# bensonlzl/spaced-kmer-sketching

Measured on AMD Instinct MI355X. Metric: k-mers hashed/s + genome-pairs ANI/s at 1/2/4/8 MI355X; % HBM roofline, higher is better.
Workload: dtype u64; 1 GPU; config3: 1x3 Gb multi-contig genome per GPU, spaced seed w=31/k=21 (mask seed 0), FracMinHash 1/1000; builds_in_flight=3, genome_bytes=3000000024, windows_per_genome=2999036400, sketch_size=2998764, parallelism=genome-sharded x1

## Files before the change

### include/sks.h

```cpp
#ifndef SKS_H
#define SKS_H

#include <stddef.h>
#include <stdint.h>

#ifdef __cplusplus
extern "C" {
#endif

#define SKS_ABI_VERSION 3

typedef enum sks_status {
  SKS_OK = 0,
  SKS_E_ARG = 1,
  SKS_E_HIP = 2,
  SKS_E_IO = 3,
  SKS_E_NOMEM = 4,
  SKS_E_UNSUPPORTED = 5,
  SKS_E_LENGTH = 6
} sks_status;

typedef enum sks_policy_kind {
  SKS_FRAC_MOD = 0,
  SKS_BOTTOM_S = 1
// ... 172 lines not shown
int sks_ani_matrix(sks_ctx* ctx, const int32_t* d_counts, uint32_t n, int kmer_num_ones, double* d_cont,
                   double* d_ani);
int sks_ani_rows(sks_ctx* ctx, const int32_t* d_counts, uint32_t n, uint32_t row_begin, uint32_t row_end,
                 int kmer_num_ones, double* d_cont, double* d_ani);
int sks_ani_tiles(sks_ctx* ctx, const int32_t* d_packed, const uint32_t* d_tiles, uint64_t n_tiles, uint32_t n,
                  const int32_t* d_sizes, int kmer_num_ones, double* d_ani);

int sks_fasta_parse_device(sks_ctx* ctx, const uint8_t* d_raw, uint64_t n_raw, uint8_t* d_stream,
                           uint64_t stream_cap, uint64_t* d_rec_end, uint64_t rec_cap,
                           uint64_t* stream_bytes, uint64_t* n_records);
int sks_ctx_last_ingress_ms(sks_ctx* ctx, float* ms);

int sks_ctx_last_intersect_ms(sks_ctx* ctx, float* ms);
int sks_ctx_set_scan_grid(sks_ctx* ctx, int grid);
enum {
  SKS_INTERSECT_AUTO = 0,
  SKS_INTERSECT_MERGE = 1,
  SKS_INTERSECT_JOIN = 2,
  SKS_INTERSECT_GLOBAL = 3
};
int sks_ctx_set_intersect_kernel(sks_ctx* ctx, int kind);
int sks_ctx_set_join_check(sks_ctx* ctx, int on);
int sks_ctx_join_check_violations(sks_ctx* ctx, uint64_t* violations);

int sks_synth_bases(sks_ctx* ctx, uint8_t* d_out, uint64_t n, uint64_t seed, uint64_t mut_seed,
                    double mut_rate, uint64_t pos_offset);

#ifdef __cplusplus
}
#endif
// ... 2 lines not shown
```

### spaced-kmer-sketching_amd/csrc/api.cpp

```cpp
#include <hip/hip_runtime.h>

#include <algorithm>
#include <cmath>
#include <cstdlib>
#include <cstring>
#include <mutex>
#include <numeric>
#include <random>
#include <string>
#include <thread>
#include <vector>

#include "sks.h"
#include "sks_api_internal.hpp"
#include "sks_hash.hpp"
#include "sks_ani.hpp"
#include "sks_internal.hpp"

namespace sks {

thread_local std::string g_last_error;

int fail(int code, const std::string& msg) {
  g_last_error = msg;
// ... 160 lines not shown
  sks::Scratch rec[3];
  sks::Scratch buf[10];
  sks::Scratch flag, pos;
  sks::Scratch meta;
  sks::Scratch iwork;
  sks::Scratch tdone;
  sks::Scratch lay;
  const uint32_t* layout_stat = nullptr;
  std::vector<uint64_t> meta_host;
  sks_timings last{};
  int grid_override = 0;
  int intersect_algo = 0;
  bool join_check = false;
  uint32_t layout_blocks_hint = 0;
  sks::Scratch root;
  uint32_t root_size = 0;
  int root_k = 0;
};

struct sks_kmer_list {
  int device = 0;
  uint32_t n = 0;
  uint64_t total = 0;
  uint64_t* d_pos = nullptr;
  uint64_t* d_bits = nullptr;
  std::vector<uint64_t> counts;
};


namespace {
// ... 151 lines not shown
      } else {
        ++i;
      }
    }
  }
  for (const CachedBlock& b : drop) {
    if (b.ready) (void)hipEventDestroy(b.ready);
    (void)hipFree(b.p);
  }
}

void release_set_arrays(sks_sketch_set* set, hipStream_t stream, bool ordered) {
  uint64_t total = 0;
  for (uint32_t v : set->sizes) total += v;
  void* arrays[3] = {set->d_data, set->d_starts, set->d_sizes};
  const size_t bytes[3] = {std::max<uint64_t>(total * set->elem_words, 1) * 8,
                           (size_t)std::max<uint32_t>(set->n, 1) * 8,
                           (size_t)std::max<uint32_t>(set->n, 1) * 4};
  for (int i = 0; i < 3; ++i) {
    if (!arrays[i]) continue;
    hipEvent_t ev = nullptr;
    if (ordered) {
      if (hipEventCreateWithFlags(&ev, hipEventDisableTiming) != hipSuccess ||
          hipEventRecord(ev, stream) != hipSuccess) {
        if (ev) (void)hipEventDestroy(ev);
        ev = nullptr;
        (void)hipGetLastError();
        (void)hipStreamSynchronize(stream);
      }
    }
    dev_release(arrays[i], bytes[i], ev);
// ... 140 lines not shown
  if (!out) return sks::fail(SKS_E_ARG, "sks_ctx_create: null out");
  *out = nullptr;
  int n = 0;
  hipError_t e = hipGetDeviceCount(&n);
  if (e != hipSuccess || n == 0)
    return sks::fail(SKS_E_HIP, std::string("sks_ctx_create: no HIP device available (the engine has "
                                            "no CPU path): hipGetDeviceCount -> ") +
                                    hipGetErrorString(e) + ", " + std::to_string(n) + " devices");
  if (device < 0 || device >= n) return sks::fail(SKS_E_ARG, "sks_ctx_create: bad device index");
  DeviceGuard g(device);
  sks_ctx* c = new (std::nothrow) sks_ctx();
  if (!c) return sks::fail(SKS_E_NOMEM, "sks_ctx_create: out of memory");
  c->device = device;
  c->stream = reinterpret_cast<hipStream_t>(stream);
  for (sks::Scratch* sc : {&c->ingress, &c->tmp, &c->rec[0], &c->rec[1], &c->rec[2], &c->flag,
                           &c->pos, &c->meta, &c->iwork, &c->tdone, &c->lay, &c->root})
    sc->owner = &c->stream;
  for (auto& b : c->buf) b.owner = &c->stream;
  if (hipEventCreate(&c->ev_begin) != hipSuccess || hipEventCreate(&c->ev_end) != hipSuccess ||
      hipEventCreate(&c->ev_s0) != hipSuccess || hipEventCreate(&c->ev_s1) != hipSuccess ||
      hipEventCreate(&c->ev_i0) != hipSuccess || hipEventCreate(&c->ev_i1) != hipSuccess) {
    delete c;
    return sks::fail(SKS_E_HIP, "sks_ctx_create: hipEventCreate failed");
  }
#define SKS_CALL_HOOK(tu) \
  if (e == hipSuccess) e = sks::code_object_hook_##tu(c->stream);
  e = hipSuccess;
  SKS_TU_LIST(SKS_CALL_HOOK)
#undef SKS_CALL_HOOK
  if (e != hipSuccess) {
    delete c;
// ... 5 lines not shown

int sks_ctx_destroy(sks_ctx* c) {
  if (!c) return SKS_OK;
  DeviceGuard g(c->device);
  (void)hipStreamSynchronize(c->stream);
  c->tmp.release();
  for (auto& r : c->rec) r.release();
  for (auto& b : c->buf) b.release();
  c->flag.release();
  c->pos.release();
  c->meta.release();
  c->iwork.release();
  c->tdone.release();
  c->lay.release();
  c->root.release();
  c->ingress.release();
  trim_device_cache(c->device);
  (void)hipEventDestroy(c->ev_begin);
  (void)hipEventDestroy(c->ev_end);
  (void)hipEventDestroy(c->ev_s0);
  (void)hipEventDestroy(c->ev_s1);
  if (c->ev_i0) (void)hipEventDestroy(c->ev_i0);
  if (c->ev_i1) (void)hipEventDestroy(c->ev_i1);
  delete c;
  return SKS_OK;
}

int sks_ctx_device(const sks_ctx* c) { return c ? c->device : -1; }

int sks_ctx_set_stream(sks_ctx* c, void* stream) {
// ... 12 lines not shown
  SKS_HIP(hipStreamSynchronize(c->stream));
  return SKS_OK;
}

int sks_ctx_last_timings(const sks_ctx* c, sks_timings* out) {
  if (!c || !out) return sks::fail(SKS_E_ARG, "sks_ctx_last_timings: null argument");
  *out = c->last;
  return SKS_OK;
}

int sks_ctx_set_scan_grid(sks_ctx* c, int grid) {
  if (!c) return sks::fail(SKS_E_ARG, "null ctx");
  c->grid_override = grid;
  return SKS_OK;
}

int sks_ctx_set_intersect_kernel(sks_ctx* c, int kind) {
  if (!c) return sks::fail(SKS_E_ARG, "null ctx");
  if (kind < SKS_INTERSECT_AUTO || kind > SKS_INTERSECT_GLOBAL)
    return sks::fail(SKS_E_ARG, "sks_ctx_set_intersect_kernel: unknown kernel");
  c->intersect_algo = kind;
  return SKS_OK;
}

int sks_ctx_set_layout_blocks_hint(sks_ctx* c, uint32_t blocks) {
  if (!c) return sks::fail(SKS_E_ARG, "sks_ctx_set_layout_blocks_hint: null ctx");
  c->layout_blocks_hint = blocks;
  return SKS_OK;
}

// ... 407 lines not shown
  tm.total_ms = tot;
  tm.post_ms = tot - ms;
  set->elem_words = 1;
  set->sizes = {(uint32_t)size};
  set->starts = {0};
  set->windows = {windows};
  set->window = S.w;
  set->mask[0] = S.mask_lo;
  set->mask[1] = S.mask_hi;
  set->policy = S.pol;
  c->last = tm;
  *out = set;
  return SKS_OK;
}

int validate_build(const char* fn, sks_ctx* c, const uint8_t* d_seq, uint64_t n_bytes,
                   const uint64_t* seg_off, uint32_t n_seg, int window, const uint64_t mask[2],
                   const sks_policy* policy) {
  const std::string f(fn);
  if (!c || !mask || !policy || (!seg_off && n_seg)) return sks::fail(SKS_E_ARG, f + ": null argument");
  if (window < 1 || window > 64)
    return sks::fail(SKS_E_ARG, f + ": window must be in [1, 64] (MAX_KMER_LENGTH)");
  if (policy->kind != SKS_FRAC_MOD && policy->kind != SKS_BOTTOM_S)
    return sks::fail(SKS_E_ARG, f + ": unknown policy kind");
  if (policy->flavour != 0 && policy->flavour != 1)
    return sks::fail(SKS_E_ARG, f + ": unknown hash flavour");
  if (policy->param == 0) return sks::fail(SKS_E_ARG, f + ": policy param must be > 0");
  {
    const int bits = 2 * window;
    uint64_t lo_allowed = bits >= 64 ? ~0ull : ((1ull << bits) - 1);
// ... 19 lines not shown
                     uint32_t n_seg, int window, const uint64_t mask[2], const sks_policy* policy,
                     sks_sketch_set** out) {
  if (!out) return sks::fail(SKS_E_ARG, "sks_sketch_build: null argument");
  *out = nullptr;
  SKS_TRY(validate_build("sks_sketch_build", c, d_seq, n_bytes, seg_off, n_seg, window, mask, policy));

  DeviceGuard guard(c->device);
  hipStream_t st = c->stream;
  BuildState S{c, window, window > 32, window > 32 ? 2 : 1, mask[0], mask[1], *policy,
               sks::fmh_const(mask[0], mask[1], window, policy->nonce, policy->flavour), {}};
  if (policy->kind == SKS_FRAC_MOD) S.dt = sks::make_div_test(policy->param);
  const bool bottom = policy->kind == SKS_BOTTOM_S;
  const double alpha = 1.0 + 10.0 / std::sqrt((double)policy->param) + 1.0 / (double)policy->param;

  sks_timings tm{};
  SKS_HIP(hipEventRecord(c->ev_begin, st));

  std::vector<uint64_t> thresh_g(n_seg, ~0ull), cap_g(n_seg), windows_g(n_seg, 0);
  std::vector<uint64_t> final_size(n_seg, ~0ull);
  for (uint32_t g = 0; g < n_seg; ++g) {
    const uint64_t L = seg_off[g + 1] - seg_off[g];
    double expect;
    if (!bottom) {
      expect = (double)L / (double)policy->param;
    } else {
      double want = alpha * (double)policy->param;
      if ((double)L <= want) {
        thresh_g[g] = ~0ull;
        expect = (double)L;
      } else {
// ... 5 lines not shown
    double cap = expect + 6.0 * std::sqrt(expect) + 4096.0;
    cap_g[g] = (uint64_t)std::min<double>(cap, (double)L + 1.0);
  }

  if (bottom && !S.wide && n_seg == 1 && getenv("SKS_NO_FAST_BOTTOM") == nullptr) {
    const uint64_t L = seg_off[1] - seg_off[0];
    const double expect = std::min<double>((double)L, alpha * (double)policy->param);
    const uint64_t cap = std::min<uint64_t>(cap_g[0], (uint64_t)(expect + 8.0 * std::sqrt(expect) + 256.0));
    if (L > 0 && cap <= sks::bottom_fused_capacity()) {
      const int rc = build_bottom_single(S, d_seq, seg_off, thresh_g[0], cap, tm, out);
      if (rc != kFastFallback) return rc;
      tm = sks_timings{};
    }
  }

  std::vector<PassOut> passes;
  std::vector<uint32_t> pending(n_seg);
  std::iota(pending.begin(), pending.end(), 0);
  int guard_passes = 0;
  while (!pending.empty()) {
    if (++guard_passes > 64) {
      free_passes(passes);
      return sks::fail(SKS_E_HIP, "sks_sketch_build: selection did not converge");
    }
    const uint32_t m = (uint32_t)pending.size();
    std::vector<uint64_t> beg(m), end(m), tp(m + 1, 0), thr(m), cap(m), ooff(m);
    uint64_t total_cap = 0;
    for (uint32_t i = 0; i < m; ++i) {
      uint32_t g = pending[i];
      beg[i] = seg_off[g];
      end[i] = seg_off[g + 1];
      tp[i + 1] = tp[i] + sks::scan_tiles_for(end[i] - beg[i]);
      thr[i] = thresh_g[g];
      cap[i] = cap_g[g];
      ooff[i] = total_cap;
      total_cap += cap[i];
    }
    const uint64_t n_tiles = tp[m];
    for (int r = 0; r < (bottom && S.wide ? 3 : (bottom || S.wide ? 2 : 1)); ++r)
      SKS_HIP(c->rec[r].reserve(std::max<uint64_t>(total_cap, 1) * sizeof(uint64_t)));
    MetaArena arena(c);
    size_t o_beg = arena.add(beg), o_end = arena.add(end), o_tp = arena.add(tp),
           o_thr = arena.add(thr), o_cap = arena.add(cap), o_off = arena.add(ooff),
           o_cnt = arena.add_zero(m), o_win = arena.add_zero(m), o_queue = arena.add_zero(1);
    SKS_TRY(arena.upload());

    const sks::ScanParams p = scan_params(S, d_seq, arena, o_beg, o_end, o_tp, o_thr, o_cap, o_off, o_cnt, o_win,
                                          m, n_tiles, o_queue);

    SKS_HIP(hipEventRecord(c->ev_s0, st));
    SKS_HIP(sks::launch_scan(p, bottom ? sks::kModeBottom : sks::kModeFrac, policy->flavour,
                             S.wide, c->device, st, c->grid_override));
    SKS_HIP(hipEventRecord(c->ev_s1, st));
    tm.scan_launches += n_tiles ? 1 : 0;
    if (o_win != o_cnt + m + 1) return sks::fail(SKS_E_HIP, "sks_sketch_build: arena layout");
    std::vector<uint64_t> cw(2 * (m + 1));
    SKS_HIP(sks::pinned_d2h(cw.data(), arena.ptr(o_cnt), cw.size() * sizeof(uint64_t), st));
    std::vector<uint64_t> counts(cw.begin(), cw.begin() + m), wins(cw.begin() + (m + 1), cw.begin() + (m + 1) + m);
    float ms = 0;
    SKS_HIP(hipEventElapsedTime(&ms, c->ev_s0, c->ev_s1));
    tm.scan_ms += ms;

    std::vector<uint32_t> ok, next;
    for (uint32_t i = 0; i < m; ++i) {
      tm.survivors += counts[i];
      if (counts[i] > cap[i]) {
        cap_g[pending[i]] = counts[i];
        next.push_back(pending[i]);
      } else {
        ok.push_back(i);
        windows_g[pending[i]] = wins[i];
      }
    }
    std::vector<uint32_t> retry_local;
    std::vector<uint64_t> fsz(m, ~0ull);
    int rc = post_process(S, pending, ooff, counts, thr, ok, passes, retry_local, fsz);
// ... 869 lines not shown
```

### spaced-kmer-sketching_amd/csrc/post.hip

```cpp
#include <hip/hip_runtime.h>

#include <algorithm>
#include <cstdio>
#include <cstring>
#include <rocprim/rocprim.hpp>
#include <rocprim/block/block_radix_sort.hpp>

#include "sks_hash.hpp"
#include "sks_internal.hpp"

namespace sks {

hipError_t Scratch::reserve(size_t n) {
  if (n <= bytes) return hipSuccess;
  const size_t grown = bytes + bytes / 2;
  if (ptr) {
    if (owner) {
      cache_release_after(ptr, bytes, *owner);
    } else {
      (void)hipDeviceSynchronize();
      (void)hipFree(ptr);
    }
  }
  ptr = nullptr;
// ... 674 lines not shown
  uint32_t eq_rank = block_excl_scan((uint32_t)__builtin_popcount(eq_m), wsum);
  uint32_t keep_m = lt_m;
#pragma unroll
  for (uint32_t j = 0; j < ITEMS; ++j)
    if ((eq_m >> j) & 1u) keep_m |= (eq_rank++ < sel.kk ? 1u : 0u) << j;
  uint32_t pos = block_excl_scan((uint32_t)__builtin_popcount(keep_m), wsum);
  uint64_t* skept = reinterpret_cast<uint64_t*>(smem);
#pragma unroll
  for (uint32_t j = 0; j < ITEMS; ++j)
    if ((keep_m >> j) & 1u) skept[pos++] = k[j];
  __syncthreads();
  for (uint32_t i = tid; i < (uint32_t)lim; i += kSelB) dst[i] = runs_expand(skept[i], runs);
  FSTAMP(7);
}

template <int FLAVOUR>
__global__ void k_fmh_narrow(uint64_t* __restrict__ keys, uint64_t n, uint64_t kconst) {
  const uint64_t i = (uint64_t)blockIdx.x * kB + threadIdx.x;
  if (i < n) keys[i] = hash_bitset128<FLAVOUR>(keys[i], 0) ^ kconst;
}

}

hipError_t seg_sort_keys(const uint64_t* keys_in, uint64_t* keys_out, uint64_t total,
                         const std::vector<uint64_t>& host_off, const uint64_t* d_off, int end_bit,
                         Scratch& tmp, hipStream_t s) {
  return sort_impl<false>(keys_in, keys_out, nullptr, nullptr, total, host_off, d_off, end_bit,
                          tmp, s);
}

// ... 237 lines not shown
      fprintf(stderr, "[k_bottom_fused stamps] n_seg %u max_cnt %llu: zero %llu count %llu scatter %llu isort %llu "
              "hash %llu distinct %llu select %llu write %llu\n", n_seg, (unsigned long long)max_cnt, h[0], h[1],
              h[2], h[3], h[4], h[5], h[6], h[7]);
    }
#endif
    return hipGetLastError();
  };
  if (max_cnt <= kSelB * 8)
    return flavour == 0 ? go(k_bottom_fused<0, 8>, fuse_lds<8>()) : go(k_bottom_fused<1, 8>, fuse_lds<8>());
  if (max_cnt <= kSelB * 12)
    return flavour == 0 ? go(k_bottom_fused<0, 12>, fuse_lds<12>())
                        : go(k_bottom_fused<1, 12>, fuse_lds<12>());
  return flavour == 0 ? go(k_bottom_fused<0, 16>, fuse_lds<16>()) : go(k_bottom_fused<1, 16>, fuse_lds<16>());
}

hipError_t launch_iota(uint64_t* out, uint64_t n, hipStream_t s) {
  if (n == 0) return hipSuccess;
  hipLaunchKernelGGL(k_iota, dim3(grid_for(n)), dim3(kB), 0, s, out, n);
  return hipGetLastError();
}

hipError_t launch_gather(const uint64_t* src, const uint64_t* idx, uint64_t n, uint64_t* out,
                         hipStream_t s) {
  if (n == 0) return hipSuccess;
  hipLaunchKernelGGL(k_gather, dim3(grid_for(n)), dim3(kB), 0, s, src, idx, n, out);
  return hipGetLastError();
}

hipError_t launch_interleave(const uint64_t* lo, const uint64_t* hi, uint64_t n, uint64_t* out,
                             hipStream_t s) {
// ... 9 lines not shown
```

### spaced-kmer-sketching_amd/csrc/sks_api_internal.hpp

```cpp
#pragma once
#include <cstdint>
#include <string>
#include <vector>

#include "sks.h"

struct sks_sketch_set {
  int device = 0;
  int elem_words = 1;
  uint32_t n = 0;
  uint64_t* d_data = nullptr;
  uint64_t* d_starts = nullptr;
  uint32_t* d_sizes = nullptr;
  std::vector<uint32_t> sizes;
  std::vector<uint64_t> starts;
  std::vector<uint64_t> windows;
  int window = 0;
  uint64_t mask[2] = {0, 0};
  sks_policy policy{};
  std::vector<std::string> names;
};

namespace sks {

int fail(int code, const std::string& msg);

inline uint8_t nucleotide_code(uint8_t ch) {
  switch (ch) {
// ... 39 lines not shown
```

### spaced-kmer-sketching_amd/csrc/sks_internal.hpp

```cpp
#pragma once
#include <hip/hip_runtime.h>

#include <cstdint>
#include <string>
#include <vector>

namespace sks {

hipError_t pinned_d2h(void* dst, const void* src, size_t bytes, hipStream_t s);
hipError_t pinned_h2d(void* dst, const void* src, size_t bytes, hipStream_t s);
size_t pinned_pool_size();

hipError_t cache_alloc(void** p, size_t bytes);
void cache_release_after(void* p, size_t bytes, hipStream_t s);

constexpr int kModeFrac = 0;
constexpr int kModeBottom = 1;
constexpr int kModeList = 2;

struct ScanParams {
  const uint8_t* seq;
  const uint64_t* seg_begin;
  const uint64_t* seg_end;
  const uint64_t* tile_prefix;
// ... 39 lines not shown
  uint32_t n = 0;
  uint64_t mask = 0;
  uint64_t mv[6] = {0, 0, 0, 0, 0, 0};
};
BitRuns bit_runs(uint64_t mask);
hipError_t launch_bits_expand(uint64_t* keys, uint64_t n, const BitRuns& runs, hipStream_t s);
constexpr uint64_t kBottomOverflow = ~1ull;
uint32_t bottom_fused_capacity();
hipError_t launch_bottom_fused(uint64_t* rec, const uint64_t* d_src_off, const uint64_t* d_cnt,
                               const uint64_t* d_retry_ok, const uint64_t* d_dst_off,
                               uint32_t n_seg, uint64_t max_cnt, uint64_t s_param, int key_bits,
                               const BitRuns& runs, uint64_t kconst, int flavour, uint64_t* out,
                               uint64_t* d_res, hipStream_t s, const uint64_t* d_cap = nullptr,
                               uint32_t* set_sizes = nullptr, uint64_t* set_starts = nullptr);

hipError_t compact_regions(const uint64_t* src, uint64_t* dst, const uint64_t* d_src_off,
                           const uint64_t* d_dst_off, uint32_t n_seg, uint64_t max_len,
                           hipStream_t s, const BitRuns* pack = nullptr, int tag_shift = -1);
int seg_tag_bits(uint32_t n_seg);
hipError_t launch_seg_ids(uint64_t* out, const uint64_t* d_off, uint32_t n_seg, uint64_t max_len, hipStream_t s);

hipError_t seg_unique_scan(const uint64_t* keys, const uint64_t* keys2, uint64_t total,
                           uint64_t max_len, const uint64_t* d_off, uint32_t n_seg, uint32_t* d_flag,
                           uint64_t* d_pos, uint64_t* d_uniq, Scratch& tmp, hipStream_t s);
hipError_t sort_unique_u64(const uint64_t* in, uint64_t n, uint64_t* out, uint64_t* n_out,
                           Scratch& tmp, hipStream_t s);
hipError_t sort_unique_u128(const uint64_t* in, uint64_t n, uint64_t* out, uint64_t* n_out,
                            Scratch& tmp, hipStream_t s);
hipError_t seg_unique_scatter(const uint64_t* vals, const uint64_t* vals2, uint64_t total,
                              uint64_t max_len, const uint64_t* d_off, uint32_t n_seg,
// ... 112 lines not shown
```

### spaced-kmer-sketching_amd/sksffi.py

```python
import ctypes as C
import os

import numpy as np

PKG_DIR = os.path.dirname(os.path.abspath(__file__))
LIB_PATH = os.environ.get("SKS_LIB") or os.path.join(PKG_DIR, "lib", "libsks.so")

SKS_FRAC_MOD = 0
SKS_BOTTOM_S = 1
INTERSECT_AUTO, INTERSECT_MERGE, INTERSECT_JOIN, INTERSECT_GLOBAL = 0, 1, 2, 3
FLAVOUR_BOOST_MIX = 0
FLAVOUR_BOOST_LEGACY = 1


SKS_OK, SKS_E_ARG, SKS_E_HIP, SKS_E_IO, SKS_E_NOMEM, SKS_E_UNSUPPORTED, SKS_E_LENGTH = range(7)


class SksError(RuntimeError):
    def __init__(self, code, msg):
        super().__init__(f"sks error {code}: {msg}")
        self.code = code


class Policy(C.Structure):
    _fields_ = [("kind", C.c_int32), ("flavour", C.c_int32), ("param", C.c_uint64),
# ... 24 lines not shown
    "sks_sketch_set_copy", "sks_sketch_set_export", "sks_intersect_pairs", "sks_intersect_all",
    "sks_synth_bases", "sks_intersect_sym", "sks_intersect_sym_tiles",
    "sks_ctx_last_intersect_ms", "sks_ctx_set_scan_grid", "sks_ctx_set_intersect_kernel", "sks_join_layout_log_b", "sks_sketch_union", "sks_sketch_union_wide",
    "sks_join_layout_capacity", "sks_join_layout_build", "sks_intersect_sym_layout", "sks_fasta_parse_device",
    "sks_ctx_last_ingress_ms", "sks_kmer_list_build", "sks_kmer_list_free", "sks_kmer_list_total",
    "sks_kmer_list_counts", "sks_kmer_list_device_positions", "sks_kmer_list_device_bits",
    "sks_kmer_list_copy", "sks_ctx_device", "sks_sketch_set_info", "sks_sketch_set_set_names",
    "sks_sketch_set_name", "sks_sketch_set_save", "sks_sketch_set_load", "sks_sketch_set_concat",
    "sks_intersect_layout_tiles",
    "sks_join_layout_bounds", "sks_join_layout_groups", "sks_join_layout_boff_words",
    "sks_ctx_set_join_check", "sks_ctx_join_check_violations", "sks_intersect_layout_pair_tiles",
    "sks_sketch_set_export_csr", "sks_ani_matrix", "sks_ani_rows", "sks_ani_tiles",
    "sks_intersect_layout_ani", "sks_host_alloc", "sks_host_free", "sks_join_layout_stat_copy",
    "sks_sketches_export", "sks_all_pairs_ani", "sks_windows_dense", "sks_windows_dense_row_words",
    "sks_join_layout_bounds_for_mask", "sks_layout_tiles_ani",
]

_lib = None


def lib():
    global _lib
    if _lib is not None:
        return _lib
    if not os.path.exists(LIB_PATH):
        raise ImportError(f"libsks.so not built ({LIB_PATH}); run __graft_entry__.build()")
    try:
        import torch
    except ImportError:
        pass
# ... 17 lines not shown
    L.sks_fasta_num_records.argtypes = [vp]
    L.sks_fasta_num_records.restype = C.c_uint64
    L.sks_fasta_record.argtypes = [vp, C.c_uint64, C.POINTER(vp), u64p]
    L.sks_fasta_stream.argtypes = [vp]
    L.sks_fasta_stream.restype = vp
    L.sks_fasta_stream_bytes.argtypes = [vp]
    L.sks_fasta_stream_bytes.restype = C.c_uint64
    L.sks_fasta_runs.argtypes = [vp, vp, vp, u64p, u64p]
    L.sks_ctx_create.argtypes = [C.c_int, vp, C.POINTER(vp)]
    L.sks_ctx_destroy.argtypes = [vp]
    L.sks_ctx_set_stream.argtypes = [vp, vp]
    L.sks_ctx_synchronize.argtypes = [vp]
    L.sks_ctx_last_timings.argtypes = [vp, C.POINTER(Timings)]
    L.sks_ctx_set_scan_grid.argtypes = [vp, C.c_int]
    L.sks_ctx_set_intersect_kernel.argtypes = [vp, C.c_int]
    L.sks_sketch_union.argtypes = [vp, vp, C.c_uint64, vp, u64p]
    L.sks_sketch_union_wide.argtypes = [vp, vp, C.c_uint64, vp, u64p]
    L.sks_join_layout_log_b.argtypes = [C.c_uint32]
    L.sks_join_layout_log_b.restype = C.c_uint32
    L.sks_join_layout_capacity.argtypes = []
    L.sks_join_layout_capacity.restype = C.c_uint32
    L.sks_join_layout_build.argtypes = [vp, vp, vp, vp, C.c_int, C.c_uint32, C.c_uint64, C.c_uint32, vp,
                                        vp, vp, vp, vp, C.POINTER(C.c_uint32)]
    L.sks_join_layout_bounds.argtypes = [vp, vp, vp, vp, C.c_int, C.c_uint32, C.c_uint32, vp]
    L.sks_join_layout_groups.argtypes = [C.c_uint32]
    L.sks_join_layout_groups.restype = C.c_uint32
    L.sks_join_layout_boff_words.argtypes = [C.c_uint32]
    L.sks_join_layout_boff_words.restype = C.c_uint32
    L.sks_intersect_sym_layout.argtypes = [vp, C.c_uint32, C.c_uint32, C.c_int, vp, vp, vp, vp, C.c_uint64,
                                           C.c_uint64, vp]
# ... 222 lines not shown
class Context:
    def __init__(self, device=0, stream=None):
        h = C.c_void_p()
        check(lib().sks_ctx_create(device, C.c_void_p(stream) if stream else None, C.byref(h)))
        self.h = h
        self.device = device
        self.stream = stream or 0

    def set_stream(self, stream):
        check(lib().sks_ctx_set_stream(self.h, C.c_void_p(stream) if stream else None))
        self.stream = stream or 0

    def set_scan_grid(self, grid):
        check(lib().sks_ctx_set_scan_grid(self.h, grid))

    def sketch_union(self, d_in, n, d_out, elem_words=1):
        k = C.c_uint64(0)
        fn = lib().sks_sketch_union if elem_words == 1 else lib().sks_sketch_union_wide
        check(fn(self.h, C.c_void_p(d_in), n, C.c_void_p(d_out), C.byref(k)))
        return int(k.value)

    def join_layout_build(self, data_ptr, starts_ptr, sizes_ptr, n, log_b, out_vals, out_masks,
                          out_boff, out_bstart, stat=True, total=None, bounds=None, elem_words=1):
        mx = C.c_uint32(0)
        check(lib().sks_join_layout_build(self.h, C.c_void_p(data_ptr), C.c_void_p(starts_ptr),
                                          C.c_void_p(sizes_ptr), elem_words, n,
                                          (1 << 64) - 1 if total is None else int(total), log_b,
                                          C.c_void_p(bounds) if bounds else None,
                                          C.c_void_p(out_vals), C.c_void_p(out_masks), C.c_void_p(out_boff),
                                          C.c_void_p(out_bstart), C.byref(mx) if stat else None))
# ... 294 lines not shown
```

Before: 708.8 billion k-mers/s.

## Add fused bucket-partition sort-unique post path for single-segment FracMinHash builds

Adds a specialised post-processing pipeline for single-segment narrow FracMinHash builds. Survivors are partitioned into key-range buckets, each bucket is sorted and deduplicated in LDS, and the results are gathered into the output set. This replaces the general multi-step post pass and avoids host round trips between stages. If a bucket overflows or the survivor cap is exceeded, it falls back to the general path, which risks doing the work twice; it also adds persistent state scratch and new tuning knobs.

```diff
diff --git a/include/sks.h b/include/sks.h
--- a/include/sks.h
+++ b/include/sks.h
@@ -210,6 +210,18 @@
 int sks_ctx_last_intersect_ms(sks_ctx* ctx, float* ms);
 int sks_ctx_set_scan_grid(sks_ctx* ctx, int grid);
 enum {
+  SKS_FRAC_POST_AUTO = 0,
+  SKS_FRAC_POST_GENERAL = 1,
+  SKS_FRAC_POST_FUSED = 2
+};
+int sks_ctx_set_frac_post(sks_ctx* ctx, int mode, uint32_t bucket_capacity, uint32_t buckets);
+enum {
+  SKS_BUILD_PATH_GENERAL = 0,
+  SKS_BUILD_PATH_FUSED = 1,
+  SKS_BUILD_PATH_FUSED_THEN_GENERAL_POST = 2
+};
+int sks_ctx_last_build_path(const sks_ctx* ctx);
+enum {
   SKS_INTERSECT_AUTO = 0,
   SKS_INTERSECT_MERGE = 1,
   SKS_INTERSECT_JOIN = 2,
diff --git a/spaced-kmer-sketching_amd/csrc/api.cpp b/spaced-kmer-sketching_amd/csrc/api.cpp
--- a/spaced-kmer-sketching_amd/csrc/api.cpp
+++ b/spaced-kmer-sketching_amd/csrc/api.cpp
@@ -198,6 +198,12 @@
   bool join_check = false;
   uint32_t layout_blocks_hint = 0;
   sks::Scratch root;
+  sks::Scratch fstate;
+  bool fstate_clean = false;
+  int frac_mode = SKS_FRAC_POST_AUTO;
+  uint32_t frac_bucket_cap = 0;
+  uint32_t frac_buckets = 0;
+  int last_path = SKS_BUILD_PATH_GENERAL;
   uint32_t root_size = 0;
   int root_k = 0;
 };
@@ -379,7 +385,7 @@
   uint64_t total = 0;
   for (uint32_t v : set->sizes) total += v;
   void* arrays[3] = {set->d_data, set->d_starts, set->d_sizes};
-  const size_t bytes[3] = {std::max<uint64_t>(total * set->elem_words, 1) * 8,
+  const size_t bytes[3] = {std::max<size_t>(std::max<uint64_t>(total * set->elem_words, 1) * 8, set->data_bytes),
                            (size_t)std::max<uint32_t>(set->n, 1) * 8,
                            (size_t)std::max<uint32_t>(set->n, 1) * 4};
   for (int i = 0; i < 3; ++i) {
@@ -550,7 +556,7 @@
   c->device = device;
   c->stream = reinterpret_cast<hipStream_t>(stream);
   for (sks::Scratch* sc : {&c->ingress, &c->tmp, &c->rec[0], &c->rec[1], &c->rec[2], &c->flag,
-                           &c->pos, &c->meta, &c->iwork, &c->tdone, &c->lay, &c->root})
+                           &c->pos, &c->meta, &c->iwork, &c->tdone, &c->lay, &c->root, &c->fstate})
     sc->owner = &c->stream;
   for (auto& b : c->buf) b.owner = &c->stream;
   if (hipEventCreate(&c->ev_begin) != hipSuccess || hipEventCreate(&c->ev_end) != hipSuccess ||
@@ -586,6 +592,7 @@
   c->tdone.release();
   c->lay.release();
   c->root.release();
+  c->fstate.release();
   c->ingress.release();
   trim_device_cache(c->device);
   (void)hipEventDestroy(c->ev_begin);
@@ -628,6 +635,19 @@
   c->grid_override = grid;
   return SKS_OK;
 }
+
+int sks_ctx_set_frac_post(sks_ctx* c, int mode, uint32_t bucket_capacity, uint32_t buckets) {
+  if (!c) return sks::fail(SKS_E_ARG, "sks_ctx_set_frac_post: null ctx");
+  if (mode != SKS_FRAC_POST_AUTO && mode != SKS_FRAC_POST_GENERAL && mode != SKS_FRAC_POST_FUSED)
+    return sks::fail(SKS_E_ARG, "sks_ctx_set_frac_post: unknown mode");
+  if (buckets & (buckets - 1)) return sks::fail(SKS_E_ARG, "sks_ctx_set_frac_post: buckets must be a power of two");
+  c->frac_mode = mode;
+  c->frac_bucket_cap = bucket_capacity;
+  c->frac_buckets = buckets;
+  return SKS_OK;
+}
+
+int sks_ctx_last_build_path(const sks_ctx* c) { return c ? c->last_path : -1; }
 
 int sks_ctx_set_intersect_kernel(sks_ctx* c, int kind) {
   if (!c) return sks::fail(SKS_E_ARG, "null ctx");
@@ -1065,6 +1085,120 @@
   return SKS_OK;
 }
 
+int frac_plan_log_b(const sks_ctx* c, uint64_t cap) {
+  const uint64_t per = sks::frac_bucket_capacity() / 4;
+  const uint64_t need = (std::max<uint64_t>(cap, 1) + per - 1) / per;
+  int lb = 0;
+  while ((1ull << lb) < need) ++lb;
+  if (lb > (int)sks::frac_max_log_buckets()) return -1;
+  if (c->frac_buckets) {
+    int fb = 0;
+    while ((1u << fb) < c->frac_buckets) ++fb;
+    lb = std::min(lb, fb);
+  }
+  return lb;
+}
+
+constexpr int kFastPostFallback = -2;
+
+int build_frac_single(BuildState& S, const uint8_t* d_seq, const uint64_t* seg_off, uint64_t cap, int log_b,
+                      sks_timings& tm, sks_sketch_set** out, uint64_t* survivors_out, uint64_t* windows_out) {
+  sks_ctx* c = S.c;
+  hipStream_t st = c->stream;
+  const uint64_t n_tiles = sks::scan_tiles_for(seg_off[1] - seg_off[0]);
+  const uint32_t bucket_cap = c->frac_bucket_cap
+                                  ? std::min<uint32_t>(c->frac_bucket_cap, sks::frac_bucket_capacity())
+                                  : sks::frac_bucket_capacity();
+  const uint64_t slots = std::max<uint64_t>(cap, 1);
+  SKS_HIP(c->rec[0].reserve(slots * sizeof(uint64_t)));
+  SKS_HIP(c->buf[0].reserve(((uint64_t)bucket_cap << log_b) * sizeof(uint64_t)));
+  SKS_HIP(c->fstate.reserve(sks::frac_state_bytes()));
+  if (!c->fstate_clean) SKS_HIP(hipMemsetAsync(c->fstate.ptr, 0, sks::frac_state_bytes(), st));
+  c->fstate_clean = false;
+  MetaArena arena(c);
+  const size_t o_beg = arena.add({seg_off[0]}), o_end = arena.add({seg_off[1]}), o_tp = arena.add({0, n_tiles}),
+               o_thr = arena.add({~0ull}), o_cap = arena.add({cap}), o_off = arena.add({0}),
+               o_cnt = arena.add_zero(1), o_win = arena.add_zero(1), o_res = arena.add_zero(2),
+               o_queue = arena.add_zero(1);
+  if (o_win != o_cnt + 2 || o_res != o_win + 2) return sks::fail(SKS_E_HIP, "sks_sketch_build: arena layout");
+  SKS_TRY(arena.upload());
+  sks_sketch_set* set = new (std::nothrow) sks_sketch_set();
+  if (!set) return sks::fail(SKS_E_NOMEM, "sks_sketch_build: out of memory");
+  set->device = c->device;
+  set->n = 1;
+  int rc = alloc_u64(&set->d_data, slots, &set->data_bytes);
+  if (rc == SKS_OK) rc = alloc_u64(&set->d_starts, 1);
+  if (rc == SKS_OK && dev_alloc(reinterpret_cast<void**>(&set->d_sizes), sizeof(uint32_t)) != hipSuccess)
+    rc = sks::fail(SKS_E_HIP, "sks_sketch_build: device allocation failed");
+  auto drop = [&]() {
+    dev_release(set->d_data, set->data_bytes);
+    dev_release(set->d_starts, 8);
+    dev_release(set->d_sizes, 8);
+    delete set;
+  };
+  if (rc != SKS_OK) {
+    drop();
+    return rc;
+  }
+  const sks::ScanParams p =
+      scan_params(S, d_seq, arena, o_beg, o_end, o_tp, o_thr, o_cap, o_off, o_cnt, o_win, 1, n_tiles, o_queue);
+  const sks::BitRuns runs = sks::bit_runs(S.mask_lo);
+  const int kb = std::max(1, __builtin_popcountll(S.mask_lo));
+  hipError_t e = hipEventRecord(c->ev_s0, st);
+  if (e == hipSuccess) e = sks::launch_scan(p, sks::kModeFrac, S.pol.flavour, false, c->device, st, c->grid_override);
+  if (e == hipSuccess) e = hipEventRecord(c->ev_s1, st);
+  if (e == hipSuccess)
+    e = sks::launch_frac_fused(reinterpret_cast<uint64_t*>(c->rec[0].ptr), arena.ptr(o_cnt), arena.ptr(o_cap), slots,
+                               kb, runs, (uint32_t)log_b, bucket_cap, col(c, 0),
+                               reinterpret_cast<uint32_t*>(c->fstate.ptr), set->d_data, set->d_sizes, set->d_starts,
+                               arena.ptr(o_res), st);
+  if (e == hipSuccess) {
+    c->fstate_clean = true;
+    e = hipEventRecord(c->ev_end, st);
+  }
+  uint64_t h[6] = {0, 0, 0, 0, 0, 0};
+  if (e == hipSuccess) e = sks::pinned_d2h(h, arena.ptr(o_cnt), sizeof h, st);
+  if (e != hipSuccess) {
+    (void)hipStreamSynchronize(st);
+    c->fstate_clean = false;
+    drop();
+    return sks::fail(SKS_E_HIP, std::string("sks_sketch_build: ") + hipGetErrorString(e));
+  }
+  const uint64_t survivors = h[0], windows = h[2], size = h[4], status = h[5];
+  float ms = 0, tot = 0;
+  (void)hipEventElapsedTime(&ms, c->ev_s0, c->ev_s1);
+  (void)hipEventElapsedTime(&tot, c->ev_begin, c->ev_end);
+  tm.scan_ms = ms;
+  tm.scan_launches = n_tiles ? 1 : 0;
+  tm.survivors = survivors;
+  if (survivors > cap || size > survivors) {
+    drop();
+    *survivors_out = survivors;
+    return kFastFallback;
+  }
+  if (status != 0) {
+    drop();
+    *survivors_out = survivors;
+    *windows_out = windows;
+    return kFastPostFallback;
+  }
+  tm.windows = windows;
+  tm.total_ms = tot;
+  tm.post_ms = tot - ms;
+  set->elem_words = 1;
+  set->sizes = {(uint32_t)size};
+  set->starts = {0};
+  set->windows = {windows};
+  set->window = S.w;
+  set->mask[0] = S.mask_lo;
+  set->mask[1] = S.mask_hi;
+  set->policy = S.pol;
+  c->last = tm;
+  c->last_path = SKS_BUILD_PATH_FUSED;
+  *out = set;
+  return SKS_OK;
+}
+
 int validate_build(const char* fn, sks_ctx* c, const uint8_t* d_seq, uint64_t n_bytes,
                    const uint64_t* seg_off, uint32_t n_seg, int window, const uint64_t mask[2],
                    const sks_policy* policy) {
@@ -1114,6 +1248,7 @@
   const double alpha = 1.0 + 10.0 / std::sqrt((double)policy->param) + 1.0 / (double)policy->param;
 
   sks_timings tm{};
+  c->last_path = SKS_BUILD_PATH_GENERAL;
   SKS_HIP(hipEventRecord(c->ev_begin, st));
 
   std::vector<uint64_t> thresh_g(n_seg, ~0ull), cap_g(n_seg), windows_g(n_seg, 0);
@@ -1149,6 +1284,24 @@
     }
   }
 
+  bool prescan = false;
+  uint64_t pre_survivors = 0, pre_windows = 0;
+  if (!bottom && !S.wide && n_seg == 1 && c->frac_mode != SKS_FRAC_POST_GENERAL &&
+      (c->frac_mode == SKS_FRAC_POST_FUSED || getenv("SKS_NO_FRAC_FUSED") == nullptr)) {
+    const int log_b = frac_plan_log_b(c, cap_g[0]);
+    if (log_b >= 0) {
+      const int rc = build_frac_single(S, d_seq, seg_off, cap_g[0], log_b, tm, out, &pre_survivors, &pre_windows);
+      if (rc == kFastPostFallback) {
+        prescan = true;
+        c->last_path = SKS_BUILD_PATH_FUSED_THEN_GENERAL_POST;
+      } else if (rc != kFastFallback) {
+        return rc;
+      } else {
+        cap_g[0] = std::max(cap_g[0], pre_survivors);
+      }
+    }
+  }
+
   std::vector<PassOut> passes;
   std::vector<uint32_t> pending(n_seg);
   std::iota(pending.begin(), pending.end(), 0);
@@ -1172,29 +1325,38 @@
       total_cap += cap[i];
     }
     const uint64_t n_tiles = tp[m];
-    for (int r = 0; r < (bottom && S.wide ? 3 : (bottom || S.wide ? 2 : 1)); ++r)
-      SKS_HIP(c->rec[r].reserve(std::max<uint64_t>(total_cap, 1) * sizeof(uint64_t)));
-    MetaArena arena(c);
-    size_t o_beg = arena.add(beg), o_end = arena.add(end), o_tp = arena.add(tp),
-           o_thr = arena.add(thr), o_cap = arena.add(cap), o_off = arena.add(ooff),
-           o_cnt = arena.add_zero(m), o_win = arena.add_zero(m), o_queue = arena.add_zero(1);
-    SKS_TRY(arena.upload());
-
-    const sks::ScanParams p = scan_params(S, d_seq, arena, o_beg, o_end, o_tp, o_thr, o_cap, o_off, o_cnt, o_win,
-                                          m, n_tiles, o_queue);
-
-    SKS_HIP(hipEventRecord(c->ev_s0, st));
-    SKS_HIP(sks::launch_scan(p, bottom ? sks::kModeBottom : sks::kModeFrac, policy->flavour,
-                             S.wide, c->device, st, c->grid_override));
-    SKS_HIP(hipEventRecord(c->ev_s1, st));
-    tm.scan_launches += n_tiles ? 1 : 0;
-    if (o_win != o_cnt + m + 1) return sks::fail(SKS_E_HIP, "sks_sketch_build: arena layout");
-    std::vector<uint64_t> cw(2 * (m + 1));
-    SKS_HIP(sks::pinned_d2h(cw.data(), arena.ptr(o_cnt), cw.size() * sizeof(uint64_t), st));
-    std::vector<uint64_t> counts(cw.begin(), cw.begin() + m), wins(cw.begin() + (m + 1), cw.begin() + (m + 1) + m);
-    float ms = 0;
-    SKS_HIP(hipEventElapsedTime(&ms, c->ev_s0, c->ev_s1));
-    tm.scan_ms += ms;
+    std::vector<uint64_t> counts, wins;
+    if (prescan) {
+      prescan = false;
+      counts = {pre_survivors};
+      wins = {pre_windows};
+      tm.survivors = 0;
+    } else {
+      for (int r = 0; r < (bottom && S.wide ? 3 : (bottom || S.wide ? 2 : 1)); ++r)
+        SKS_HIP(c->rec[r].reserve(std::max<uint64_t>(total_cap, 1) * sizeof(uint64_t)));
+      MetaArena arena(c);
+      size_t o_beg = arena.add(beg), o_end = arena.add(end), o_tp = arena.add(tp),
+             o_thr = arena.add(thr), o_cap = arena.add(cap), o_off = arena.add(ooff),
+             o_cnt = arena.add_zero(m), o_win = arena.add_zero(m), o_queue = arena.add_zero(1);
+      SKS_TRY(arena.upload());
+
+      const sks::ScanParams p = scan_params(S, d_seq, arena, o_beg, o_end, o_tp, o_thr, o_cap, o_off, o_cnt, o_win,
+                                            m, n_tiles, o_queue);
+
+      SKS_HIP(hipEventRecord(c->ev_s0, st));
+      SKS_HIP(sks::launch_scan(p, bottom ? sks::kModeBottom : sks::kModeFrac, policy->flavour,
+                               S.wide, c->device, st, c->grid_override));
+      SKS_HIP(hipEventRecord(c->ev_s1, st));
+      tm.scan_launches += n_tiles ? 1 : 0;
+      if (o_win != o_cnt + m + 1) return sks::fail(SKS_E_HIP, "sks_sketch_build: arena layout");
+      std::vector<uint64_t> cw(2 * (m + 1));
+      SKS_HIP(sks::pinned_d2h(cw.data(), arena.ptr(o_cnt), cw.size() * sizeof(uint64_t), st));
+      counts.assign(cw.begin(), cw.begin() + m);
+      wins.assign(cw.begin() + (m + 1), cw.begin() + (m + 1) + m);
+      float ms = 0;
+      SKS_HIP(hipEventElapsedTime(&ms, c->ev_s0, c->ev_s1));
+      tm.scan_ms += ms;
+    }
 
     std::vector<uint32_t> ok, next;
     for (uint32_t i = 0; i < m; ++i) {
diff --git a/spaced-kmer-sketching_amd/csrc/post.hip b/spaced-kmer-sketching_amd/csrc/post.hip
--- a/spaced-kmer-sketching_amd/csrc/post.hip
+++ b/spaced-kmer-sketching_amd/csrc/post.hip
@@ -712,6 +712,234 @@
   FSTAMP(7);
 }
 
+constexpr int kFracB = 256;
+constexpr int kFracWaves = kFracB / 64;
+constexpr uint32_t kFracItems = 16;
+constexpr uint32_t kFracCap = kFracB * kFracItems;
+constexpr int kFracPartB = 1024;
+constexpr uint32_t kFracPartTile = 1u << 14;
+constexpr int kFracSubLog = 11;
+constexpr uint32_t kFracSub = 1u << kFracSubLog;
+constexpr uint32_t kFracSubPer = kFracSub / kFracB;
+constexpr uint32_t kFracSubMax = 32;
+constexpr uint32_t kFracMaxLogB = 14;
+constexpr uint32_t kFracStateCounts = 1u << kFracMaxLogB;
+constexpr uint32_t kFracStateStatus = 2u << kFracMaxLogB;
+
+__global__ __launch_bounds__(kFracPartB) void k_frac_partition(const uint64_t* __restrict__ rec,
+                                                               const uint64_t* __restrict__ seg_count,
+                                                               const uint64_t* __restrict__ seg_cap,
+                                                               const BitRuns runs, int shift, uint32_t n_buckets,
+                                                               uint32_t bucket_cap, uint64_t* __restrict__ regions,
+                                                               uint32_t* __restrict__ state) {
+  extern __shared__ uint32_t s_cur[];
+  const uint64_t n = seg_count[0];
+  if (n > seg_cap[0]) return;
+  const uint64_t rows = (n + kFracPartB - 1) / kFracPartB;
+  const uint64_t share = (rows + gridDim.x - 1) / gridDim.x * kFracPartB;
+  const uint64_t lo = min((uint64_t)blockIdx.x * share, n), hi = min(lo + share, n);
+  if (lo >= hi) return;
+  auto bucket_of = [&](uint64_t key) {
+    const uint64_t top = shift < 64 ? key >> shift : 0ull;
+    return (uint32_t)min(top, (uint64_t)(n_buckets - 1));
+  };
+  for (uint32_t b = threadIdx.x; b < n_buckets; b += kFracPartB) s_cur[b] = 0;
+  __syncthreads();
+#pragma unroll 4
+  for (uint64_t i = lo + threadIdx.x; i < hi; i += kFracPartB) atomicAdd(&s_cur[bucket_of(runs_pack(rec[i], runs))], 1u);
+  __syncthreads();
+  for (uint32_t b = threadIdx.x; b < n_buckets; b += kFracPartB) {
+    const uint32_t c = s_cur[b];
+    if (c) s_cur[b] = atomicAdd(&state[b], c);
+  }
+  __syncthreads();
+  bool over = false;
+#pragma unroll 4
+  for (uint64_t i = lo + threadIdx.x; i < hi; i += kFracPartB) {
+    const uint64_t key = runs_pack(rec[i], runs);
+    const uint32_t b = bucket_of(key);
+    const uint32_t slot = atomicAdd(&s_cur[b], 1u);
+    if (slot < bucket_cap) regions[(uint64_t)b * bucket_cap + slot] = key;
+    else over = true;
+  }
+  if (over) atomicOr(&state[kFracStateStatus], (uint32_t)kFracStatusBucket);
+}
+
+__device__ __forceinline__ uint32_t frac_excl_scan(uint32_t v, uint32_t* wsum, uint32_t* total) {
+  const int lane = threadIdx.x & 63, wave = threadIdx.x >> 6;
+  uint32_t inc = v;
+#pragma unroll
+  for (int o = 1; o < 64; o <<= 1) {
+    const uint32_t t = __shfl_up(inc, o, 64);
+    if (lane >= o) inc += t;
+  }
+  if (lane == 63) wsum[wave] = inc;
+  __syncthreads();
+  uint32_t before = inc - v, all = 0;
+#pragma unroll
+  for (int w = 0; w < kFracWaves; ++w) {
+    before += w < wave ? wsum[w] : 0u;
+    all += wsum[w];
+  }
+  __syncthreads();
+  *total = all;
+  return before;
+}
+
+template <uint32_t ITEMS>
+__device__ __forceinline__ void frac_sort_body(uint64_t* __restrict__ reg, uint32_t n, uint32_t b,
+                                               uint32_t* __restrict__ state, const BitRuns& runs, int shift,
+                                               uint64_t* skeys, uint32_t* sbin, uint32_t* wsum, uint32_t* wmax) {
+  const int tid = threadIdx.x;
+  uint64_t k[ITEMS];
+#pragma unroll
+  for (uint32_t j = 0; j < ITEMS; ++j) {
+    const uint32_t i = j * kFracB + tid;
+    k[j] = i < n ? reg[i] : ~0ull;
+  }
+  const uint64_t low = shift >= 64 ? ~0ull : (1ull << shift) - 1;
+  const int sub_shift = shift > kFracSubLog ? shift - kFracSubLog : 0;
+  auto sub_of = [&](uint64_t key) { return (uint32_t)min((key & low) >> sub_shift, (uint64_t)(kFracSub - 1)); };
+#pragma unroll
+  for (uint32_t j = 0; j < ITEMS; ++j)
+    if (j * kFracB + tid < n) atomicAdd(&sbin[sub_of(k[j])], 1u);
+  __syncthreads();
+  uint32_t cb[kFracSubPer], sum = 0, mx = 0;
+#pragma unroll
+  for (uint32_t q = 0; q < kFracSubPer; ++q) {
+    cb[q] = sbin[tid * kFracSubPer + q];
+    sum += cb[q];
+    mx = cb[q] > mx ? cb[q] : mx;
+  }
+#pragma unroll
+  for (int o = 32; o > 0; o >>= 1) mx = max(mx, (uint32_t)__shfl_xor(mx, o, 64));
+  if ((tid & 63) == 0) wmax[tid >> 6] = mx;
+  uint32_t total;
+  const uint32_t excl = frac_excl_scan(sum, wsum, &total);
+  uint32_t bmax = 0;
+#pragma unroll
+  for (int w = 0; w < kFracWaves; ++w) bmax = wmax[w] > bmax ? wmax[w] : bmax;
+  if (bmax > kFracSubMax) {
+    if (tid == 0) {
+      state[kFracStateCounts + b] = 0;
+      atomicOr(&state[kFracStateStatus], (uint32_t)kFracStatusCrowd);
+    }
+    return;
+  }
+  {
+    uint32_t run = excl;
+#pragma unroll
+    for (uint32_t q = 0; q < kFracSubPer; ++q) {
+      sbin[tid * kFracSubPer + q] = run;
+      run += cb[q];
+    }
+  }
+  __syncthreads();
+#pragma unroll
+  for (uint32_t j = 0; j < ITEMS; ++j)
+    if (j * kFracB + tid < n) skeys[atomicAdd(&sbin[sub_of(k[j])], 1u)] = k[j];
+  __syncthreads();
+  {
+    uint32_t st = excl;
+#pragma unroll 1
+    for (uint32_t q = 0; q < kFracSubPer; ++q) {
+      const uint32_t c = cb[q];
+      for (uint32_t i = 1; i < c; ++i) {
+        const uint64_t key = skeys[st + i];
+        uint32_t j = i;
+        while (j > 0 && skeys[st + j - 1] > key) {
+          skeys[st + j] = skeys[st + j - 1];
+          --j;
+        }
+        skeys[st + j] = key;
+      }
+      st += c;
+    }
+  }
+  __syncthreads();
+  const uint64_t before = tid ? skeys[tid * ITEMS - 1] : 0ull;
+  uint32_t first_m = 0;
+#pragma unroll
+  for (uint32_t j = 0; j < ITEMS; ++j) {
+    const uint32_t i = tid * ITEMS + j;
+    k[j] = skeys[i];
+    const bool first = i < n && (i == 0 || k[j] != (j ? k[j - 1] : before));
+    first_m |= (first ? 1u : 0u) << j;
+  }
+  uint32_t distinct;
+  uint32_t pos = frac_excl_scan((uint32_t)__builtin_popcount(first_m), wsum, &distinct);
+#pragma unroll
+  for (uint32_t j = 0; j < ITEMS; ++j)
+    if ((first_m >> j) & 1u) skeys[pos++] = k[j];
+  __syncthreads();
+  for (uint32_t i = tid; i < distinct; i += kFracB) reg[i] = runs_expand(skeys[i], runs);
+  if (tid == 0) state[kFracStateCounts + b] = distinct;
+}
+
+__global__ __launch_bounds__(kFracB) void k_frac_sort_unique(uint64_t* __restrict__ regions,
+                                                             uint32_t* __restrict__ state, const BitRuns runs,
+                                                             int shift, uint32_t bucket_cap) {
+  __shared__ uint64_t skeys[kFracCap];
+  __shared__ uint32_t sbin[kFracSub];
+  __shared__ uint32_t wsum[kFracWaves], wmax[kFracWaves];
+  __shared__ uint32_t s_n;
+  const uint32_t b = blockIdx.x;
+  const int tid = threadIdx.x;
+  uint32_t* counts = state + kFracStateCounts;
+  if (tid == 0) {
+    s_n = state[b];
+    state[b] = 0;
+  }
+#pragma unroll
+  for (uint32_t q = 0; q < kFracSubPer; ++q) sbin[tid * kFracSubPer + q] = 0;
+  __syncthreads();
+  const uint32_t n = s_n;
+  if (n == 0 || n > bucket_cap) {
+    if (tid == 0) {
+      counts[b] = 0;
+      if (n) atomicOr(&state[kFracStateStatus], (uint32_t)kFracStatusBucket);
+    }
+    return;
+  }
+  uint64_t* reg = regions + (uint64_t)b * bucket_cap;
+  if (n <= 4 * kFracB) frac_sort_body<4>(reg, n, b, state, runs, shift, skeys, sbin, wsum, wmax);
+  else if (n <= 8 * kFracB) frac_sort_body<8>(reg, n, b, state, runs, shift, skeys, sbin, wsum, wmax);
+  else frac_sort_body<kFracItems>(reg, n, b, state, runs, shift, skeys, sbin, wsum, wmax);
+}
+
+__global__ __launch_bounds__(kFracB) void k_frac_gather(const uint64_t* __restrict__ regions,
+                                                        uint32_t* __restrict__ state, uint32_t n_buckets,
+                                                        uint32_t bucket_cap, uint64_t out_cap,
+                                                        uint64_t* __restrict__ out, uint32_t* __restrict__ set_sizes,
+                                                        uint64_t* __restrict__ set_starts,
+                                                        uint64_t* __restrict__ res) {
+  __shared__ uint32_t wsum[kFracWaves];
+  const uint32_t b = blockIdx.x;
+  const int tid = threadIdx.x;
+  const uint32_t* counts = state + kFracStateCounts;
+  uint32_t part = 0;
+  for (uint32_t j = tid; j < b; j += kFracB) part += counts[j];
+#pragma unroll
+  for (int o = 32; o > 0; o >>= 1) part += __shfl_xor(part, o, 64);
+  if ((tid & 63) == 0) wsum[tid >> 6] = part;
+  __syncthreads();
+  uint64_t prefix = 0;
+#pragma unroll
+  for (int w = 0; w < kFracWaves; ++w) prefix += wsum[w];
+  const uint32_t cnt = counts[b];
+  const uint64_t* reg = regions + (uint64_t)b * bucket_cap;
+  for (uint32_t i = tid; i < cnt; i += kFracB)
+    if (prefix + i < out_cap) out[prefix + i] = reg[i];
+  if (b == n_buckets - 1 && tid == 0) {
+    const uint64_t total = prefix + cnt;
+    set_sizes[0] = (uint32_t)total;
+    set_starts[0] = 0;
+    res[0] = total;
+    res[1] = state[kFracStateStatus];
+    state[kFracStateStatus] = 0;
+  }
+}
+
 template <int FLAVOUR>
 __global__ void k_fmh_narrow(uint64_t* __restrict__ keys, uint64_t n, uint64_t kconst) {
   const uint64_t i = (uint64_t)blockIdx.x * kB + threadIdx.x;
@@ -979,6 +1207,29 @@
   return flavour == 0 ? go(k_bottom_fused<0, 16>, fuse_lds<16>()) : go(k_bottom_fused<1, 16>, fuse_lds<16>());
 }
 
+uint32_t frac_bucket_capacity() { return kFracCap; }
+uint32_t frac_max_log_buckets() { return kFracMaxLogB; }
+size_t frac_state_bytes() { return (size_t)(kFracStateStatus + 2) * sizeof(uint32_t); }
+
+hipError_t launch_frac_fused(const uint64_t* rec, const uint64_t* d_cnt, const uint64_t* d_cap, uint64_t cap,
+                             int key_bits, const BitRuns& runs, uint32_t log_b, uint32_t bucket_cap,
+                             uint64_t* regions, uint32_t* state, uint64_t* out, uint32_t* set_sizes,
+                             uint64_t* set_starts, uint64_t* d_res, hipStream_t s) {
+  if (log_b > kFracMaxLogB || bucket_cap == 0 || bucket_cap > kFracCap || key_bits < 1 || key_bits > 64)
+    return hipErrorInvalidValue;
+  const uint32_t n_buckets = 1u << log_b;
+  const int shift = key_bits > (int)log_b ? key_bits - (int)log_b : 0;
+  const uint64_t tiles = (std::max<uint64_t>(cap, 1) + kFracPartTile - 1) / kFracPartTile;
+  hipLaunchKernelGGL(k_frac_partition, dim3((unsigned)std::min<uint64_t>(tiles, 256)), dim3(kFracPartB),
+                     n_buckets * sizeof(uint32_t), s, rec, d_cnt, d_cap, runs, shift, n_buckets, bucket_cap, regions,
+                     state);
+  hipLaunchKernelGGL(k_frac_sort_unique, dim3(n_buckets), dim3(kFracB), 0, s, regions, state, runs, shift,
+                     bucket_cap);
+  hipLaunchKernelGGL(k_frac_gather, dim3(n_buckets), dim3(kFracB), 0, s, regions, state, n_buckets, bucket_cap,
+                     cap, out, set_sizes, set_starts, d_res);
+  return hipGetLastError();
+}
+
 hipError_t launch_iota(uint64_t* out, uint64_t n, hipStream_t s) {
   if (n == 0) return hipSuccess;
   hipLaunchKernelGGL(k_iota, dim3(grid_for(n)), dim3(kB), 0, s, out, n);
diff --git a/spaced-kmer-sketching_amd/csrc/sks_api_internal.hpp b/spaced-kmer-sketching_amd/csrc/sks_api_internal.hpp
--- a/spaced-kmer-sketching_amd/csrc/sks_api_internal.hpp
+++ b/spaced-kmer-sketching_amd/csrc/sks_api_internal.hpp
@@ -12,6 +12,7 @@
   uint64_t* d_data = nullptr;
   uint64_t* d_starts = nullptr;
   uint32_t* d_sizes = nullptr;
+  size_t data_bytes = 0;
   std::vector<uint32_t> sizes;
   std::vector<uint64_t> starts;
   std::vector<uint64_t> windows;
diff --git a/spaced-kmer-sketching_amd/csrc/sks_internal.hpp b/spaced-kmer-sketching_amd/csrc/sks_internal.hpp
--- a/spaced-kmer-sketching_amd/csrc/sks_internal.hpp
+++ b/spaced-kmer-sketching_amd/csrc/sks_internal.hpp
@@ -77,6 +77,16 @@
                                uint64_t* d_res, hipStream_t s, const uint64_t* d_cap = nullptr,
                                uint32_t* set_sizes = nullptr, uint64_t* set_starts = nullptr);
 
+constexpr uint64_t kFracStatusBucket = 1;
+constexpr uint64_t kFracStatusCrowd = 2;
+uint32_t frac_bucket_capacity();
+uint32_t frac_max_log_buckets();
+size_t frac_state_bytes();
+hipError_t launch_frac_fused(const uint64_t* rec, const uint64_t* d_cnt, const uint64_t* d_cap, uint64_t cap,
+                             int key_bits, const BitRuns& runs, uint32_t log_b, uint32_t bucket_cap,
+                             uint64_t* regions, uint32_t* state, uint64_t* out, uint32_t* set_sizes,
+                             uint64_t* set_starts, uint64_t* d_res, hipStream_t s);
+
 hipError_t compact_regions(const uint64_t* src, uint64_t* dst, const uint64_t* d_src_off,
                            const uint64_t* d_dst_off, uint32_t n_seg, uint64_t max_len,
                            hipStream_t s, const BitRuns* pack = nullptr, int tag_shift = -1);
diff --git a/spaced-kmer-sketching_amd/sksffi.py b/spaced-kmer-sketching_amd/sksffi.py
--- a/spaced-kmer-sketching_amd/sksffi.py
+++ b/spaced-kmer-sketching_amd/sksffi.py
@@ -9,6 +9,8 @@
 SKS_FRAC_MOD = 0
 SKS_BOTTOM_S = 1
 INTERSECT_AUTO, INTERSECT_MERGE, INTERSECT_JOIN, INTERSECT_GLOBAL = 0, 1, 2, 3
+FRAC_POST_AUTO, FRAC_POST_GENERAL, FRAC_POST_FUSED = 0, 1, 2
+BUILD_PATH_GENERAL, BUILD_PATH_FUSED, BUILD_PATH_FUSED_THEN_GENERAL_POST = 0, 1, 2
 FLAVOUR_BOOST_MIX = 0
 FLAVOUR_BOOST_LEGACY = 1
 
@@ -63,6 +65,7 @@
     "sks_intersect_layout_ani", "sks_host_alloc", "sks_host_free", "sks_join_layout_stat_copy",
     "sks_sketches_export", "sks_all_pairs_ani", "sks_windows_dense", "sks_windows_dense_row_words",
     "sks_join_layout_bounds_for_mask", "sks_layout_tiles_ani",
+    "sks_ctx_set_frac_post", "sks_ctx_last_build_path",
 ]
 
 _lib = None
@@ -110,6 +113,8 @@
     L.sks_ctx_last_timings.argtypes = [vp, C.POINTER(Timings)]
     L.sks_ctx_set_scan_grid.argtypes = [vp, C.c_int]
     L.sks_ctx_set_intersect_kernel.argtypes = [vp, C.c_int]
+    L.sks_ctx_set_frac_post.argtypes = [vp, C.c_int, C.c_uint32, C.c_uint32]
+    L.sks_ctx_last_build_path.argtypes = [vp]
     L.sks_sketch_union.argtypes = [vp, vp, C.c_uint64, vp, u64p]
     L.sks_sketch_union_wide.argtypes = [vp, vp, C.c_uint64, vp, u64p]
     L.sks_join_layout_log_b.argtypes = [C.c_uint32]
@@ -362,6 +367,12 @@
     def set_scan_grid(self, grid):
         check(lib().sks_ctx_set_scan_grid(self.h, grid))
 
+    def set_frac_post(self, mode=0, bucket_capacity=0, buckets=0):
+        check(lib().sks_ctx_set_frac_post(self.h, mode, bucket_capacity, buckets))
+
+    def last_build_path(self):
+        return int(lib().sks_ctx_last_build_path(self.h))
+
     def sketch_union(self, d_in, n, d_out, elem_words=1):
         k = C.c_uint64(0)
         fn = lib().sks_sketch_union if elem_words == 1 else lib().sks_sketch_union_wide
```

Result: faster. 727.0 billion k-mers/s (median of 6 runs) (+2.6%).
